# Isabella98Liu/DG-Mesh

Hardware: AMD Instinct MI355X
Metric: train-step iters/sec (800x800, ~100k Gaussians) (higher is better)
Workload: dtype f32 (f16x3p split products, fp32 accumulate); 1 GPU; D-NeRF jumpingjacks-like cfg2: 800x800, P=100000 Gaussians, deformation MLP on (deform + deform_back, is_blender), 1 frame per rank per step, fixed P (no densification inside the timed region); output heads of both networks scaled x0.01 so that the deformation field is small as after convergence (default init triples every splat's extent); P=100000, W=800, H=800, num_rendered=2808497, visible=95520, mlp_impl=hip, parallelism=dp1 (frame-parallel, flat-bucket all-reduce 27.8 MB)

## Files before the change

dg-mesh_amd/csrc/mlp.hip:

```cpp
#include <stdlib.h>
#include <string.h>

#include "dgm_common.hpp"
#include "mlp_planes.hpp"
#include "mlp_planes5.hpp"

namespace dgm {

static constexpr int MLP_W = 256;
static constexpr int MLP_EMB = 96;
static constexpr int MLP_XE = 63;
static constexpr int GM = 64, GK = 16, GAP = 66;
static constexpr int DW_ROWS = 512;
static constexpr int DW_SLAB = 128;
static constexpr int HD_ROWS = 256;

__global__ void mlp_prep_kernel(int in_features, int Kp, int emb_dim, int is_skip, const float* __restrict__ W,
                                float* __restrict__ Wt, float* __restrict__ Wd) {
    const int idx = blockIdx.x * blockDim.x + threadIdx.x;
    if (idx < Kp * MLP_W) {
        const int k = idx / MLP_W, j = idx % MLP_W;
        int src = -1;
        if (Kp == MLP_W) src = k;
        else if (k < MLP_EMB) src = k < emb_dim ? k : -1;
// ... 911 lines not shown
                dgm::prof_begin(DGM_STAGE_MLP_LAYER_FWD, st);
                P4_LAUNCH((mlp_gemm4_kernel<16, 1024, 512, 0, false, 8, true>), CfgFwdC::LDS, gx, st, a)
                dgm::prof_end(DGM_STAGE_MLP_LAYER_FWD, st);
            }
        }
    } else {
    a.A = (const unsigned char*)w.emb, a.Aexp = w.Eexp, a.Bp = w.Wt3[0], a.b_inv = w.wsc_f[0], a.bias = p->b[0];
    a.mask_out = w.mask[0], a.C = (unsigned char*)w.Y[0], a.Cexp = w.Yexp[0];
    a.Bp2 = w.Wt3[sk], a.b_inv2 = w.wsc_e, a.bias2 = p->b[sk], a.out2 = w.Cin;
    P4_LAUNCH((mlp_gemm4_kernel<6, 384, 192, 0, true, 8>), CfgL0::LDS, gx, st, a)
    a.Bp2 = nullptr, a.b_inv2 = nullptr, a.bias2 = nullptr, a.out2 = nullptr;
    for (int l = 1; l < 8; l++) {
        a.A = (const unsigned char*)w.Y[l - 1], a.Aexp = w.Yexp[l - 1], a.b_inv = w.wsc_f[l], a.bias = p->b[l];
        a.mask_out = w.mask[l], a.C = (unsigned char*)w.Y[l], a.Cexp = w.Yexp[l];
        if (l == sk) {
            a.Bp = w.Wt3[l] + (size_t)MLP_EMB * MLP_W / 4, a.cin = w.Cin;
            P4_LAUNCH((mlp_gemm4_kernel<16, 1024, 512, 2, false, 8>), CfgSkip::LDS, gx, st, a)
            a.cin = nullptr;
        } else {
            a.Bp = w.Wt3[l];
            dgm::prof_begin(DGM_STAGE_MLP_LAYER_FWD, st);
            P4_LAUNCH((mlp_gemm4_kernel<16, 1024, 512, 0, false, 8>), CfgFwd::LDS, gx, st, a)
            dgm::prof_end(DGM_STAGE_MLP_LAYER_FWD, st);
        }
    }
    }
    a.Bp2 = nullptr, a.b_inv2 = nullptr, a.bias2 = nullptr, a.out2 = nullptr, a.cin = nullptr;
    a.A = (const unsigned char*)w.Y[7], a.Aexp = w.Yexp[7], a.Bp = w.Wh4f, a.b_inv = w.wsc_hf, a.bias = p->bh;
    a.mask_out = nullptr, a.C = nullptr, a.Cexp = nullptr, a.out = out, a.ldo = p->n_out, a.n_valid = p->n_out;
    if (fold && heads_fused) {}
    else if (fold) P4_LAUNCH((mlp_gemm4_kernel<16, 1024, 512, 3, false, 1, true>), CfgHeadsC::LDS, gx, st, a)
    else P4_LAUNCH((mlp_gemm4_kernel<16, 1024, 512, 3, false, 1>), CfgHeads::LDS, gx, st, a)
    hipError_t e = hipGetLastError();
    if (e != hipSuccess) return mlp_fail(hipGetErrorString(e));
    return 0;
}

int backward_planes(const dgm_mlp_params* p, int N, const float* dOut, int temb_stride, const Ws& w, float* const* dW, float* const* db,
                    float* dWh, float* dbh, float* dtemb, hipStream_t st, const bool fold, const bool all5, const float* x_in = nullptr,
                    float* dX = nullptr) {
    const P4Plan pl = p4_plan(N);
    const int nt = pl.ntiles, gx = nt < num_cus() ? nt : num_cus();
    const int sk = p->skip_layer;
    const int EW = fold ? 64 : MLP_EMB;
    hipLaunchKernelGGL(mlp_dout4_kernel, dim3((nt + 3) / 4), dim3(256), 0, st, N, nt, p->n_out, dOut, w.Dp, w.Dexp, w.partial_hb);
    unsigned char* G = (unsigned char*)w.Ga;
    unsigned char* Gn = (unsigned char*)w.Gb;
    int *Ge = w.Gexp[0], *Gne = w.Gexp[1];
    Gemm4Args a;
    memset(&a, 0, sizeof(a));
    a.ntiles = nt, a.M = N, a.exps_limit = p4_exps_limit();
    a.A = w.Dp, a.Aexp = w.Dexp, a.Bp = w.Wh4b, a.b_inv = w.wsc_hb, a.mask_in = w.mask[7], a.C = G, a.Cexp = Ge;
    Dw4Args d;
    memset(&d, 0, sizeof(d));
    d.ntiles = nt, d.tiles_per_chunk = pl.tiles_per_chunk;
    d.X = (const unsigned char*)w.Y[7], d.Xexp = w.Yexp[7], d.G = w.Dp, d.Gexp = w.Dexp, d.partial = w.partial_h, d.chunk_stride = 0;
    d.partial_db = nullptr;
    {
        static const int mult = [] { const char* e = getenv("DGM_P4_G7_MULT"); return e ? atoi(e) : 2; }();
        const int g7 = nt < mult * num_cus() ? nt : mult * num_cus();
        if (fold) P4_LAUNCH((mlp_gemm4_kernel<1, 128, 64, 1, false, 8, true>), CfgG7C::LDS, g7, st, a)
        else P4_LAUNCH((mlp_gemm4_kernel<1, 128, 64, 1, false, 8>), CfgG7::LDS, g7, st, a)
    }
    P4_LAUNCH((mlp_dw4_kernel<8, 1, 1024, 512, 128, 64>), CfgDwH::LDS, pl.chunks, st, d)
    ReduceDwBatch rb;
    rb.emb_dim = p->emb_dim, rb.n_jobs = 0;
    int rb_blocks = 0, n_pending = 0;
    auto add_job = [&](int slot, int chunks, int db_rows, int Kp, int in_features, int dst_off, const float* partial,
                       const float* partial_db, float* dWp, float* dbp) {
        ReduceDwJob& jb = rb.job[slot];
        jb.chunks = chunks, jb.db_rows = db_rows, jb.Kp = Kp, jb.in_features = in_features, jb.nblocks = reduce_dw_blocks(Kp);
        jb.emb_rows = EW, jb.k_valid = fold ? MLP_XE : p->emb_dim;
        jb.dst_off = dst_off, jb.partial = partial, jb.partial_db = partial_db, jb.dW = dWp, jb.db = dbp;
        if (jb.nblocks > rb_blocks) rb_blocks = jb.nblocks;
    };
    int n_dw = p4_pair_split(nt, gx);
    if (n_dw > pl.chunks) n_dw = pl.chunks;
    const bool per_row_t = temb_stride != 0 && dtemb != nullptr;
    if (per_row_t && dX) return mlp_fail("mlp_backward: position gradients need a broadcast time row");
    for (int l = 7; l >= 0; l--) {
        const int Kp = l == 0 ? EW : (l == sk ? EW + MLP_W : MLP_W);
        const bool paired = n_dw > 0 && l >= 1;
        const int tpc_pair = paired ? (nt + n_dw - 1) / n_dw : 0;
        const int chunks_l = paired ? (nt + tpc_pair - 1) / tpc_pair : pl.chunks;
        if (l >= 1) {
            a.A = G, a.Aexp = Ge, a.Bp = w.Wd3[l], a.b_inv = w.wsc_d[l], a.mask_in = w.mask[l - 1], a.C = Gn, a.Cexp = Gne;
        }
        d.G = G, d.Gexp = Ge;
        if (dX && (l == sk || l == 0))
            hipLaunchKernelGGL(mlp_dx4_kernel, dim3(nt), dim3(256), 0, st, N, (const unsigned char*)G, (const int*)Ge, p->W[l],
                               layer_in(p, l), 0, MLP_XE, reinterpret_cast<float*>(w.Cin), l == 0 ? 1 : 0, x_in, dX, 0);
        if (per_row_t && (l == sk || l == 0))
            hipLaunchKernelGGL(mlp_dx4_kernel, dim3(nt), dim3(256), 0, st, N, (const unsigned char*)G, (const int*)Ge, p->W[l],
                               layer_in(p, l), MLP_XE, p->t_dim, reinterpret_cast<float*>(w.Cin), l == 0 ? 2 : 0, (const float*)nullptr,
                               dtemb, p->t_dim);
        float* part_emb = w.partial_l[l];
        float* part_trunk = w.partial_l[l] + (l == sk ? (size_t)EW * MLP_W : 0);
        size_t stride_emb = (size_t)Kp * MLP_W, stride_trunk = (size_t)Kp * MLP_W;
        if (paired && l == sk) {
            part_trunk = w.partial_l[l], stride_trunk = (size_t)MLP_W * MLP_W;
            part_emb = w.partial_l[l] + (size_t)n_dw * MLP_W * MLP_W, stride_emb = (size_t)EW * MLP_W;
        }
        if (l == 0 || l == sk) {
            d.tiles_per_chunk = pl.tiles_per_chunk;
            d.X = (const unsigned char*)w.emb, d.Xexp = w.Eexp, d.partial = part_emb, d.chunk_stride = stride_emb, d.partial_db = w.partial_db_l[l];
            if (fold) P4_LAUNCH((mlp_dw4_kernel<2, 8, 256, 128, 1024, 512>), CfgDwE64::LDS, pl.chunks, st, d)
            else P4_LAUNCH((mlp_dw4_kernel<3, 8, 384, 192, 1024, 512>), CfgDwE::LDS, pl.chunks, st, d)
        }
        if (l != 0) {
            d.tiles_per_chunk = paired ? tpc_pair : pl.tiles_per_chunk;
            d.X = (const unsigned char*)w.Y[l - 1], d.Xexp = w.Yexp[l - 1];
            d.partial = part_trunk, d.chunk_stride = stride_trunk;
            d.partial_db = l == sk ? nullptr : w.partial_db_l[l];
        }
        if (paired) {
            dgm::prof_begin(DGM_STAGE_MLP_BWD_PAIR, st);
            {
                static bool done_[DGM_MAX_DEVICES] = {false}, donec_[DGM_MAX_DEVICES] = {false};
                constexpr int LDS_PAIR = CfgBwdC::LDS > CfgDw::LDS ? CfgBwdC::LDS : CfgDw::LDS;
                if ((fold ? p4_lds_attr(mlp_bwd_pair_kernel<true>, LDS_PAIR, &donec_[current_device_slot()])
                          : p4_lds_attr(mlp_bwd_pair_kernel<false>, LDS_PAIR, &done_[current_device_slot()])) != hipSuccess)
                    return mlp_fail("mlp: cannot raise the LDS limit of mlp_bwd_pair_kernel");
                const int grid = n_dw + (gx - n_dw > 0 ? gx - n_dw : 1);
                static const int chunk_env = [] { const char* e = getenv("DGM_MLP_PAIR_CHUNKED"); return e ? atoi(e) : 1; }();
                const int chunked = (chunk_env && grid - n_dw == n_dw && (n_dw % 8) == 0) ? 1 : 0;
                if (fold) hipLaunchKernelGGL(mlp_bwd_pair_kernel<true>, dim3(grid), dim3(512), LDS_PAIR, st, a, d, n_dw, chunked);
                else hipLaunchKernelGGL(mlp_bwd_pair_kernel<false>, dim3(grid), dim3(512), LDS_PAIR, st, a, d, n_dw, chunked);
            }
            dgm::prof_end(DGM_STAGE_MLP_BWD_PAIR, st);
        } else if (l >= 1) {
            dgm::prof_begin(DGM_STAGE_MLP_LAYER_BWD, st);
            if (all5) {
                Gemm5Args b;
                memset(&b, 0, sizeof(b));
                b.ntiles = nt, b.M = N, b.exps_limit = a.exps_limit;
                b.A = a.A, b.Aexp = a.Aexp, b.Bp = a.Bp, b.b_inv = a.b_inv, b.mask_in = a.mask_in, b.C = a.C, b.Cexp = a.Cexp;
                P5_LAUNCH((mlp_gemm5_kernel<0, 1>), Cfg5Bwd::LDS, gx, st, b)
            } else if (fold)
                P4_LAUNCH((mlp_gemm4_kernel<16, 1024, 512, 1, false, 8, true>), CfgBwdC::LDS, gx, st, a)
            else
                P4_LAUNCH((mlp_gemm4_kernel<16, 1024, 512, 1, false, 8>), CfgBwd::LDS, gx, st, a)
            dgm::prof_end(DGM_STAGE_MLP_LAYER_BWD, st);
            dgm::prof_begin(DGM_STAGE_MLP_LAYER_DW, st);
            P4_LAUNCH((mlp_dw4_kernel<8, 8, 1024, 512, 1024, 512>), CfgDw::LDS, chunks_l, st, d)
            dgm::prof_end(DGM_STAGE_MLP_LAYER_DW, st);
        }
        if (paired && l == sk) {
            add_job(n_pending++, pl.chunks, 8 * pl.chunks, EW, layer_in(p, l), 0, part_emb, w.partial_db_l[l], dW[l], db[l]);
            add_job(n_pending++, chunks_l, 0, MLP_W, layer_in(p, l), p->emb_dim, part_trunk, nullptr, dW[l], nullptr);
        } else
            add_job(n_pending++, chunks_l, 8 * chunks_l, Kp, layer_in(p, l), 0, w.partial_l[l], w.partial_db_l[l], dW[l], db[l]);
        if (l >= 1) {
            unsigned char* t = G;
            G = Gn, Gn = t;
            int* te = Ge;
            Ge = Gne, Gne = te;
        }
    }
    rb.n_jobs = n_pending;
    rb.h_chunks = pl.chunks, rb.h_bchunks = nt, rb.h_nout = p->n_out, rb.h_partial_W = w.partial_h, rb.h_partial_b = w.partial_hb;
    rb.h_dW = dWh, rb.h_db = dbh;
    hipLaunchKernelGGL(mlp_reduce_dw_all_kernel, dim3(rb_blocks, rb.n_jobs + 1), dim3(256), 0, st, rb);
    if (fold) {
        FoldGradArgs f;
        f.dW[0] = dW[0], f.db[0] = db[0], f.W[0] = p->W[0], f.in_features[0] = layer_in(p, 0);
        f.dW[1] = dW[sk], f.db[1] = db[sk], f.W[1] = p->W[sk], f.in_features[1] = layer_in(p, sk);
        f.temb = w.temb_row, f.T = p->t_dim, f.dtemb = (dtemb != nullptr && !per_row_t) ? dtemb : nullptr;
        hipLaunchKernelGGL(mlp_fold_grad_kernel, dim3(f.dtemb != nullptr ? 3 : 2, p->t_dim), dim3(256), 0, st, f);
    } else if (dtemb != nullptr && !per_row_t)
        hipLaunchKernelGGL(mlp_dtemb_bcast_kernel, dim3(p->t_dim), dim3(256), 0, st, p->t_dim, db[0], p->W[0], layer_in(p, 0),
                           db[sk], p->W[sk], layer_in(p, sk), dtemb);
    hipError_t e = hipGetLastError();
    if (e != hipSuccess) return mlp_fail(hipGetErrorString(e));
    return 0;
}
}

extern "C" {

int dgm_mlp_set_gemm(int mode) {
    const int prev = g_gemm_mode;
    if (mode == 1 || mode == 3 || mode == 4 || mode == 5) g_gemm_mode = mode;
    return prev;
}

size_t dgm_mlp_workspace_bytes(int N) {
    Ws w = carve(nullptr, N > 0 ? N : 0);
    return w.bytes;
}

#ifdef P4_TIMING
int dgm_p4_timing(unsigned long long* out) {
    return (int)hipMemcpyFromSymbol(out, HIP_SYMBOL(dgm::g_p4_timing), sizeof(unsigned long long) * 256 * 8 * 16);
}
#endif

#ifdef P4_PROBE
namespace {
__global__ void p4_probe_fill_kernel(unsigned* __restrict__ p, size_t n, unsigned seed, int zero) {
    for (size_t i = blockIdx.x * (size_t)blockDim.x + threadIdx.x; i < n; i += (size_t)gridDim.x * blockDim.x) {
        unsigned x = (unsigned)i * 2654435761u + seed;
        x ^= x >> 15, x *= 0x2c1b3c6du, x ^= x >> 12;
        p[i] = zero ? 0u : (x & 0xbfffbfffu);
    }
}
}
int dgm_p4_probe(int N, int kind, int iters, int zero, void* stream) {
    hipStream_t st = (hipStream_t)stream;
    const P4Plan pl = p4_plan(N);
    const int nt = pl.ntiles, gx = nt < num_cus() ? nt : num_cus();
    static unsigned char *A = nullptr, *C = nullptr, *G = nullptr;
    static int* ex = nullptr;
    static uint4* Bp = nullptr;
    static float *binv = nullptr, *bias = nullptr, *partial = nullptr, *pdb = nullptr;
    static unsigned* mask = nullptr;
    static int cap = 0;
    const size_t rows = (size_t)nt * 32;
    if (cap < nt) {
        if (hipMalloc((void**)&A, rows * 1024) != hipSuccess || hipMalloc((void**)&C, rows * 1024) != hipSuccess ||
            hipMalloc((void**)&G, rows * 1024) != hipSuccess || hipMalloc((void**)&ex, (size_t)nt * 4 * 4) != hipSuccess ||
            hipMalloc((void**)&Bp, 16 * 4 * 256 * 16) != hipSuccess || hipMalloc((void**)&binv, 1024) != hipSuccess ||
            hipMalloc((void**)&bias, 1024) != hipSuccess || hipMalloc((void**)&mask, (size_t)nt * 1024) != hipSuccess ||
            hipMalloc((void**)&partial, (size_t)256 * 256 * 256 * 4) != hipSuccess || hipMalloc((void**)&pdb, (size_t)256 * 8 * 256 * 4) != hipSuccess)
            return mlp_fail("p4_probe: hipMalloc failed");
        cap = nt;
    }
    hipLaunchKernelGGL(p4_probe_fill_kernel, dim3(1024), dim3(256), 0, st, (unsigned*)A, rows * 256, 1u, zero);
    hipLaunchKernelGGL(p4_probe_fill_kernel, dim3(1024), dim3(256), 0, st, (unsigned*)G, rows * 256, 2u, zero);
    hipLaunchKernelGGL(p4_probe_fill_kernel, dim3(64), dim3(256), 0, st, (unsigned*)Bp, (size_t)16 * 4 * 256 * 4, 3u, zero);
    hipLaunchKernelGGL(p4_probe_fill_kernel, dim3(256), dim3(256), 0, st, mask, (size_t)nt * 256, 4u, 0);
    (void)hipMemsetAsync(ex, 0, (size_t)nt * 4 * 4, st);
    (void)hipMemsetAsync(bias, 0, 1024, st);
    const float one = 1.0f / 65536.0f;
    {
        float ones[256];
        for (int i = 0; i < 256; i++) ones[i] = one;
        (void)hipMemcpyAsync(binv, ones, sizeof(ones), hipMemcpyHostToDevice, st);
        (void)hipStreamSynchronize(st);
    }
    Gemm4Args a;
    memset(&a, 0, sizeof(a));
    a.exps_limit = 512;
    a.ntiles = nt, a.M = N, a.A = kind == 0 ? A : G, a.Aexp = ex, a.Bp = Bp, a.b_inv = binv, a.bias = bias, a.mask_in = mask,
    a.mask_out = mask + (size_t)0, a.C = C, a.Cexp = ex + nt;
    Dw4Args d;
    memset(&d, 0, sizeof(d));
    d.ntiles = nt, d.tiles_per_chunk = pl.tiles_per_chunk, d.X = A, d.Xexp = ex + 2 * nt, d.G = G, d.Gexp = ex + 3 * nt, d.partial = partial,
    d.chunk_stride = (size_t)256 * 256, d.partial_db = pdb;
    int n_dw = p4_pair_split(nt, gx);
    if (n_dw > pl.chunks) n_dw = pl.chunks;
    Gemm5Args a5;
    memset(&a5, 0, sizeof(a5));
    a5.exps_limit = 512, a5.ntiles = nt, a5.M = N, a5.A = (kind == 4) ? A : G, a5.Aexp = ex, a5.Bp = Bp, a5.b_inv = binv, a5.bias = bias;
    a5.mask_in = mask, a5.mask_out = mask, a5.C = C, a5.Cexp = ex + nt;
    for (int it = 0; it < iters; it++) {
        if (kind == 4) {
            P5_LAUNCH((mlp_gemm5_kernel<0, 0>), Cfg5Fwd::LDS, gx, st, a5)
        } else if (kind == 5) {
            P5_LAUNCH((mlp_gemm5_kernel<0, 1>), Cfg5Bwd::LDS, gx, st, a5)
        } else if (kind == 0) {
            P4_LAUNCH((mlp_gemm4_kernel<16, 1024, 512, 0, false, 8>), CfgFwd::LDS, gx, st, a)
        } else if (kind == 3) {
            P4_LAUNCH((mlp_gemm4_kernel<16, 1024, 512, 1, false, 8>), CfgBwd::LDS, gx, st, a)
        } else if (kind == 1) {
            P4_LAUNCH((mlp_dw4_kernel<8, 8, 1024, 512, 1024, 512>), CfgDw::LDS, pl.chunks, st, d)
        } else {
            if (n_dw <= 0) return mlp_fail("p4_probe: no pair split at this size");
            static bool done_[DGM_MAX_DEVICES] = {false};
            constexpr int LDS_PAIR = CfgBwd::LDS > CfgDw::LDS ? CfgBwd::LDS : CfgDw::LDS;
            if (p4_lds_attr(mlp_bwd_pair_kernel<false>, LDS_PAIR, &done_[current_device_slot()]) != hipSuccess) return mlp_fail("p4_probe: LDS attribute");
            Dw4Args dp = d;
            dp.tiles_per_chunk = (nt + n_dw - 1) / n_dw;
#ifdef P4_XCD_REDUCE
            {
                static unsigned* xs = nullptr;
                static float* xp = nullptr;
                static int gen = 0;
                if (!xs) {
                    if (hipMalloc((void**)&xs, 8 * 128) != hipSuccess || hipMalloc((void**)&xp, (size_t)8 * 65536 * 4) != hipSuccess) return mlp_fail("p4_probe: hipMalloc");
                    (void)hipMemsetAsync(xs, 0, 8 * 128, st);
                }
                dp.xsync = getenv("DGM_P4_XCD_OFF") ? nullptr : xs, dp.xpartial = xp, dp.xgen = gen++, dp.xchunks = (nt + dp.tiles_per_chunk - 1) / dp.tiles_per_chunk;
            }
#endif
            const int grid = n_dw + (gx - n_dw > 0 ? gx - n_dw : 1);
            const int chunked = (grid - n_dw == n_dw && (n_dw % 8) == 0) ? 1 : 0;
            hipLaunchKernelGGL(mlp_bwd_pair_kernel<false>, dim3(grid), dim3(512), LDS_PAIR, st, a, dp, n_dw, chunked);
        }
    }
    hipError_t e = hipGetLastError();
    if (e != hipSuccess) return mlp_fail(hipGetErrorString(e));
    return 0;
}
#endif

int dgm_mlp_describe_workspace(int N, size_t* offs, int capacity) {
    Ws w = carve(nullptr, N > 0 ? N : 0);
    const char* base = nullptr;
    const void* f[DGM_MLP_WS_FIELDS];
    int n = 0;
    f[n++] = w.emb;
    for (int l = 0; l < 8; l++) f[n++] = w.Y[l];
    for (int l = 0; l < 8; l++) f[n++] = w.mask[l];
    f[n++] = w.Ga, f[n++] = w.Gb;
    f[n++] = w.Eexp;
    for (int l = 0; l < 8; l++) f[n++] = w.Yexp[l];
    f[n++] = w.Dexp, f[n++] = w.Gexp[0], f[n++] = w.Gexp[1];
    f[n++] = w.Cin, f[n++] = w.Dp;
    for (int l = 0; l < 8; l++) f[n++] = w.partial_l[l];
    for (int l = 0; l < 8; l++) f[n++] = w.partial_db_l[l];
    for (int i = 0; i < n && i < capacity; i++) offs[i] = (size_t)((const char*)f[i] - base);
    return n;
}

int dgm_mlp_forward(const dgm_mlp_params* p, int N, const float* x, const float* temb, int temb_stride, char* workspace,
                    float* out, void* stream) {
    if (check_params(p)) return 1;
    if (N <= 0) return 0;
    if (!x || !temb || !workspace || !out) return mlp_fail("mlp_forward: NULL pointer");
    hipStream_t st = (hipStream_t)stream;
    Ws w = carve(workspace, N);
    const int mode = g_gemm_mode;
    const bool fold = (mode == 3 || mode == 5) && temb_stride == 0;
    remember_ws_mode(workspace, mode + (fold ? 16 : 0));
    if (mode >= 3) return forward_planes(p, N, x, temb, temb_stride, w, out, st, fold, fold && mode == 5);
    for (int l = 0; l < 8; l++) {
        const int Kp = layer_kp(p, l);
        const int n = (Kp > MLP_W ? Kp : MLP_W) * MLP_W;
        hipLaunchKernelGGL(mlp_prep_kernel, dim3((n + 255) / 256), dim3(256), 0, st, layer_in(p, l), Kp, p->emb_dim,
                           l == p->skip_layer ? 1 : 0, p->W[l], w.Wt[l], l >= 1 ? w.Wd[l] : nullptr);
    }
    hipLaunchKernelGGL(mlp_embed_kernel, dim3((N + 7) / 8), dim3(256), 0, st, N, x, temb, temb_stride, p->t_dim, w.emb);
    const int grid = (N + GM - 1) / GM;
    for (int l = 0; l < 8; l++) {
        const float *A1, *A2 = nullptr;
        int lda1, K1, lda2 = 0, K2 = 0;
        if (l == 0) {
            A1 = w.emb, lda1 = MLP_EMB, K1 = MLP_EMB;
        } else if (l == p->skip_layer) {
            A1 = w.emb, lda1 = MLP_EMB, K1 = MLP_EMB, A2 = w.Y[l - 1], lda2 = MLP_W, K2 = MLP_W;
        } else {
            A1 = w.Y[l - 1], lda1 = MLP_W, K1 = MLP_W;
        }
        hipLaunchKernelGGL(mlp_gemm_kernel<0>, dim3(grid, MLP_W / GN), dim3(256), 0, st, N, A1, lda1, K1, A2, lda2, K2, w.Wt[l],
                           p->b[l], w.mask[l], w.Y[l]);
    }
    hipLaunchKernelGGL(mlp_rows_small_kernel, dim3((N * 4 + 255) / 256), dim3(256), 0, st, N, p->n_out, w.Y[7], p->Wh, 1,
                       MLP_W, p->bh, out, p->n_out, 0);
    hipError_t e = hipGetLastError();
    if (e != hipSuccess) return mlp_fail(hipGetErrorString(e));
    return 0;
}

int dgm_mlp_backward(const dgm_mlp_params* p, int N, const float* dOut, int temb_stride, char* workspace, float* const* dW,
                     float* const* db, float* dWh, float* dbh, float* dtemb, void* stream) {
    return dgm_mlp_backward_dx(p, N, dOut, temb_stride, workspace, dW, db, dWh, dbh, dtemb, nullptr, nullptr, stream);
}

int dgm_mlp_backward_dx(const dgm_mlp_params* p, int N, const float* dOut, int temb_stride, char* workspace, float* const* dW,
                        float* const* db, float* dWh, float* dbh, float* dtemb, const float* x, float* dX, void* stream) {
    if (check_params(p)) return 1;
    if (N <= 0) return 0;
    if (!dOut || !workspace || !dW || !db || !dWh || !dbh) return mlp_fail("mlp_backward: NULL pointer");
    if ((x == nullptr) != (dX == nullptr)) return mlp_fail("mlp_backward: x and dX come together");
    const int mode = g_gemm_mode;
    if (dX && (mode < 3 || temb_stride != 0))
        return mlp_fail("mlp_backward: the gradient w.r.t. the positions exists in the plane arithmetic only (f16x3p, broadcast time row)");
    {
        const int fm = recall_ws_mode(workspace);
        if (fm >= 0 && (fm & 15) != mode)
// ... 84 lines not shown
```

dg-mesh_amd/csrc/mlp_planes.hpp:

```cpp
#pragma once
#include <type_traits>

#include "dgm_common.hpp"

namespace dgm {

typedef _Float16 f16x8 __attribute__((ext_vector_type(8)));
typedef _Float16 f16x2 __attribute__((ext_vector_type(2)));
typedef float f32x2 __attribute__((ext_vector_type(2)));
#ifndef DGM_F32X16_DEFINED
#define DGM_F32X16_DEFINED
typedef float f32x16 __attribute__((ext_vector_type(16)));
#endif

__device__ __forceinline__ f16x8 as_f16x8(const uint4 v) { return __builtin_bit_cast(f16x8, v); }

__device__ __forceinline__ void split2h(float a0, float a1, unsigned& h, unsigned& l) {
    const f16x2 hh = __builtin_convertvector((f32x2){a0, a1}, f16x2);
    const float r0 = a0 - (float)hh.x, r1 = a1 - (float)hh.y;
    const f16x2 ll = __builtin_convertvector((f32x2){r0, r1}, f16x2);
    h = __builtin_bit_cast(unsigned, hh);
    l = __builtin_bit_cast(unsigned, ll);
}

// ... 796 lines not shown
        if (HM.value && j + 1 < my_tiles)
            asm volatile("s_waitcnt lgkmcnt(%0)\n\ts_barrier" ::"n"((EPI == 0 ? 4 : 0) + 2 * (P4_PD < KS ? P4_PD : KS) + (COLSC ? 1 : 0)) : "memory");
        else if (HM.value && EPI == 0) asm volatile("s_waitcnt lgkmcnt(%0)\n\ts_barrier" ::"n"(4 + (COLSC ? 1 : 0)) : "memory");
        else P4_LDS_BARRIER();
        P4_T(6)
    };
    {
        const unsigned char* ps = Abuf + li * PITCH + g * 16;
#pragma unroll
        for (int i = 0; i < P4_PD && i < KS; i++) G4_FRAG(i);
    }
    typedef std::integral_constant<bool, true> T_;
    typedef std::integral_constant<bool, false> F_;
    step(T_{}, F_{}, F_{}, 0, 0);
    if (my_tiles > 1) step(T_{}, T_{}, F_{}, 1, 1);
    int ab = 2;
    for (int j = 2; j < my_tiles; j++) {
        step(T_{}, T_{}, T_{}, j, ab);
        ab = ab == 2 ? 0 : ab + 1;
    }
    if (my_tiles >= 2) step(F_{}, T_{}, T_{}, my_tiles, my_tiles % 3);
    else step(F_{}, T_{}, F_{}, my_tiles, my_tiles % 3);
    step(F_{}, F_{}, T_{}, my_tiles + 1, (my_tiles + 1) % 3);
#ifdef P4_TIMING
    if (P4_TIME_ON && lane == 0 && bx < 256) {
#pragma unroll
        for (int k = 0; k < 8; k++) g_p4_timing[(bx * 8 + wv) * 16 + k] = tacc[k];
        g_p4_timing[(bx * 8 + wv) * 16 + 8] = t_loop - t_entry;
        g_p4_timing[(bx * 8 + wv) * 16 + 9] = __builtin_amdgcn_s_memtime() - t_entry;
        g_p4_timing[(bx * 8 + wv) * 16 + 10] = t_entry;
        g_p4_timing[(bx * 8 + wv) * 16 + 11] = __builtin_amdgcn_s_memtime();
        g_p4_timing[(bx * 8 + wv) * 16 + 12] = my_tiles;
        g_p4_timing[(bx * 8 + wv) * 16 + 13] = t_p1 - t_entry;
        g_p4_timing[(bx * 8 + wv) * 16 + 14] = t_p2 - t_p1;
        g_p4_timing[(bx * 8 + wv) * 16 + 15] = t_p3 - t_p2;
    }
#endif
#undef G4_COPY
#undef G4_COPY1
#undef G4_FRAG
#undef G4_MFMA
}

template <int KS, int ROWB, int PLANEB, int EPI, bool DUAL, int NCW, bool COLSC = false>
__global__ void __launch_bounds__(512)
mlp_gemm4_kernel(const Gemm4Args a) {
    extern __shared__ __attribute__((aligned(16))) unsigned char p4_smem[];
    gemm4_body<KS, ROWB, PLANEB, EPI, DUAL, NCW, COLSC>(a, (int)blockIdx.x, (int)gridDim.x, p4_smem);
}

struct Dw4Args {
    int ntiles, tiles_per_chunk;
    const unsigned char* X;
    const int* Xexp;
    const unsigned char* G;
    const int* Gexp;
    float* partial;
    size_t chunk_stride;
    float* partial_db;
#ifdef P4_XCD_REDUCE
    unsigned* xsync;
    float* xpartial;
    int xgen, xchunks;
#endif
};

__device__ __forceinline__ int dw4_pos(int col) { return (col & ~7) | ((col ^ (col >> 3)) & 7); }
__device__ __forceinline__ unsigned dw4_dword(const uint4& v, int i) { return i == 0 ? v.x : (i == 1 ? v.y : (i == 2 ? v.z : v.w)); }
__device__ __forceinline__ float dw4_dot_ones(unsigned d, float acc) {
    const f16x2 one = {(_Float16)1.0f, (_Float16)1.0f};
    return __builtin_amdgcn_fdot2(__builtin_bit_cast(f16x2, d), one, acc, false);
}
__device__ __forceinline__ unsigned dw4_pk_mul(unsigned d, unsigned f2) {
    return __builtin_bit_cast(unsigned, __builtin_bit_cast(f16x2, d) * __builtin_bit_cast(f16x2, f2));
}

template <int MT, int NT, int XROWB, int XPLANEB, int GROWB, int GPLANEB>
struct Dw4Cfg {
    static constexpr int XK = MT * 32, GK = NT * 32;
    static constexpr int XU = 8 * XK, GU = 8 * GK;
    static constexpr int LDS = 2 * (XU + GU) * 16;
};

template <int MT, int NT, int XROWB, int XPLANEB, int GROWB, int GPLANEB>
__device__ __forceinline__ void dw4_body(const Dw4Args& a, const int chunk, unsigned char* smem) {
    using Cfg = Dw4Cfg<MT, NT, XROWB, XPLANEB, GROWB, GPLANEB>;
    constexpr int XK = Cfg::XK, GK = Cfg::GK, XU = Cfg::XU, GU = Cfg::GU;
    constexpr int XCG = XK / 8, GCG = GK / 8;
    constexpr int XB = XCG * 8, GB = GCG * 8;
    constexpr int MTW = NT == 8 ? MT : 1;
    static_assert(NT == 8 || (NT == 1 && MT == 8), "wave decomposition");
    static_assert(XB <= 256 && GB <= 256, "stager layout");
    uint4* const dw4_lds = reinterpret_cast<uint4*>(smem);
    uint4* Xs = dw4_lds;
    uint4* Gs = dw4_lds + 2 * XU;
    const int tid = threadIdx.x, lane = tid & 63, wv = __builtin_amdgcn_readfirstlane(tid >> 6);
    const int g = lane >> 5, li = lane & 31;
    const int t0 = chunk * a.tiles_per_chunk, t1 = min(a.ntiles, t0 + a.tiles_per_chunk);
    const int nst = t1 - t0;
    if (nst <= 0) return;

    int eref = 0x7fffffff;
    for (int t = t0; t < t1; t++) eref = min(eref, a.Xexp[t] + a.Gexp[t]);
    eref = __builtin_amdgcn_readfirstlane(eref);

    const bool isX = tid < XB, isG = tid >= 256 && tid < 256 + GB;
    const int st = isG ? tid - 256 : tid;
    const int ncg = isG ? GCG : XCG;
#ifndef DW4_ROWMAJOR_STAGERS
#define DW4_ROWMAJOR_STAGERS 1
#endif
    const int cg = st % ncg;
    const int pl = DW4_ROWMAJOR_STAGERS ? (st / ncg) & 1 : st / (ncg * 4);
    const int rg = DW4_ROWMAJOR_STAGERS ? st / (ncg * 2) : (st / ncg) & 3;
    const unsigned char* src = isG ? a.G + (size_t)pl * GPLANEB + cg * 16 : a.X + (size_t)pl * XPLANEB + cg * 16;
    const int srow = isG ? GROWB : XROWB;
    uint4* sdst = (isG ? Gs : Xs) + (pl * 4 + rg) * (isG ? GK : XK) + cg * 8;
    const int sbuf = isG ? GU : XU;
    const int swz = cg & 7;
    uint4 R[8];
    float cs[8];
#pragma unroll
    for (int i = 0; i < 8; i++) cs[i] = 0.f;

#define DW4_LOAD(t_)                                                                                                   \
    if (isX || isG) {                                                                                                  \
        const unsigned char* p_ = src + ((size_t)(t_) * 32 + rg * 8) * srow;                                           \
        _Pragma("unroll") for (int i_ = 0; i_ < 8; i_++) R[i_] = *reinterpret_cast<const uint4*>(p_ + (size_t)i_ * srow); \
    }
#define DW4_STORE(t_, buf_)                                                                                            \
    if (isX || isG) {                                                                                                  \
        const int et_ = a.Xexp[t_] + a.Gexp[t_];                                                                       \
        const unsigned f2_ = p4_pow2_h2(eref - et_);                                                                   \
        const bool scale_ = isX && et_ != eref;                                                                        \
        float tsum_[8];                                                                                                \
        _Pragma("unroll") for (int c_ = 0; c_ < 8; c_++) {                                                             \
            const unsigned sel_ = (c_ & 1) ? 0x07060302u : 0x05040100u;                                                \
            uint4 o_;                                                                                                  \
            o_.x = __builtin_amdgcn_perm(dw4_dword(R[1], c_ >> 1), dw4_dword(R[0], c_ >> 1), sel_);                    \
            o_.y = __builtin_amdgcn_perm(dw4_dword(R[3], c_ >> 1), dw4_dword(R[2], c_ >> 1), sel_);                    \
            o_.z = __builtin_amdgcn_perm(dw4_dword(R[5], c_ >> 1), dw4_dword(R[4], c_ >> 1), sel_);                    \
            o_.w = __builtin_amdgcn_perm(dw4_dword(R[7], c_ >> 1), dw4_dword(R[6], c_ >> 1), sel_);                    \
            if (isG && a.partial_db != nullptr) {                                                                      \
                float s_ = dw4_dot_ones(o_.x, 0.f);                                                                    \
                s_ = dw4_dot_ones(o_.y, s_), s_ = dw4_dot_ones(o_.z, s_), s_ = dw4_dot_ones(o_.w, s_);                 \
                tsum_[c_] = s_;                                                                                        \
            }                                                                                                          \
            if (scale_) o_.x = dw4_pk_mul(o_.x, f2_), o_.y = dw4_pk_mul(o_.y, f2_), o_.z = dw4_pk_mul(o_.z, f2_), o_.w = dw4_pk_mul(o_.w, f2_); \
            sdst[(buf_) * sbuf + (c_ ^ swz)] = o_;                                                                     \
        }                                                                                                              \
        if (isG && a.partial_db != nullptr) {                                                                          \
            const float ig_ = p4_pow2(-a.Gexp[t_]);                                                                    \
            _Pragma("unroll") for (int c_ = 0; c_ < 8; c_++) cs[c_] += tsum_[c_] * ig_;                                \
        }                                                                                                              \
    }

    f32x16 acc[MTW];
#pragma unroll
    for (int mt = 0; mt < MTW; mt++)
#pragma unroll
        for (int r = 0; r < 16; r++) acc[mt][r] = 0.f;

    const int gcol = NT == 8 ? wv * 32 + li : li;
    const int gpos = dw4_pos(gcol);

    DW4_LOAD(t0)
    DW4_STORE(t0, 0)
    if (nst > 1) DW4_LOAD(t0 + 1)
    __syncthreads();
    for (int s = 0; s < nst; s++) {
        const int buf = s & 1;
        if (s + 1 < nst) {
            DW4_STORE(t0 + s + 1, buf ^ 1)
            if (s + 2 < nst) DW4_LOAD(t0 + s + 2)
        }
        __builtin_amdgcn_sched_barrier(0);
        const uint4* xs = Xs + buf * XU;
        const uint4* gs = Gs + buf * GU;
#pragma unroll
        for (int kk = 0; kk < 2; kk++) {
            const int kg = 2 * kk + g;
            const f16x8 gh = as_f16x8(gs[kg * GK + gpos]), gl = as_f16x8(gs[(4 + kg) * GK + gpos]);
            if (MTW == 1) {
                const int xpos = dw4_pos(wv * 32 + li);
                const f16x8 ah = as_f16x8(xs[kg * XK + xpos]), al = as_f16x8(xs[(4 + kg) * XK + xpos]);
                acc[0] = __builtin_amdgcn_mfma_f32_32x32x16_f16(ah, gl, acc[0], 0, 0, 0);
                acc[0] = __builtin_amdgcn_mfma_f32_32x32x16_f16(al, gh, acc[0], 0, 0, 0);
                acc[0] = __builtin_amdgcn_mfma_f32_32x32x16_f16(ah, gh, acc[0], 0, 0, 0);
            } else {
#pragma unroll
                for (int mp = 0; mp < (MTW + 1) / 2; mp++) {
                    const int m0 = 2 * mp, m1 = 2 * mp + 1 < MTW ? 2 * mp + 1 : 2 * mp;
                    const int xp0 = dw4_pos(m0 * 32 + li), xp1 = dw4_pos(m1 * 32 + li);
                    const f16x8 ah0 = as_f16x8(xs[kg * XK + xp0]), al0 = as_f16x8(xs[(4 + kg) * XK + xp0]);
                    if (m1 != m0) {
                        const f16x8 ah1 = as_f16x8(xs[kg * XK + xp1]), al1 = as_f16x8(xs[(4 + kg) * XK + xp1]);
                        acc[m0] = __builtin_amdgcn_mfma_f32_32x32x16_f16(ah0, gl, acc[m0], 0, 0, 0);
                        acc[m1] = __builtin_amdgcn_mfma_f32_32x32x16_f16(ah1, gl, acc[m1], 0, 0, 0);
                        acc[m0] = __builtin_amdgcn_mfma_f32_32x32x16_f16(al0, gh, acc[m0], 0, 0, 0);
                        acc[m1] = __builtin_amdgcn_mfma_f32_32x32x16_f16(al1, gh, acc[m1], 0, 0, 0);
                        acc[m0] = __builtin_amdgcn_mfma_f32_32x32x16_f16(ah0, gh, acc[m0], 0, 0, 0);
                        acc[m1] = __builtin_amdgcn_mfma_f32_32x32x16_f16(ah1, gh, acc[m1], 0, 0, 0);
                    } else {
                        acc[m0] = __builtin_amdgcn_mfma_f32_32x32x16_f16(ah0, gl, acc[m0], 0, 0, 0);
                        acc[m0] = __builtin_amdgcn_mfma_f32_32x32x16_f16(al0, gh, acc[m0], 0, 0, 0);
                        acc[m0] = __builtin_amdgcn_mfma_f32_32x32x16_f16(ah0, gh, acc[m0], 0, 0, 0);
                    }
                }
            }
        }
        P4_LDS_BARRIER();
    }
#undef DW4_LOAD
#undef DW4_STORE

    if (NT == 8) {
        float* out = a.partial + (size_t)chunk * a.chunk_stride;
        const int col = wv * 32 + li;
#pragma unroll
        for (int mt = 0; mt < MTW; mt++) {
#pragma unroll
            for (int r = 0; r < 16; r++) {
                const int k = mt * 32 + (r & 3) + 8 * (r >> 2) + 4 * g;
                out[(size_t)k * 256 + col] = ldexpf(acc[mt][r], -eref);
            }
        }
#ifdef P4_XCD_REDUCE
        if (MT == 8 && a.xsync != nullptr) {
            const int grp = chunk & 7, member = chunk >> 3;
            const int members = (a.xchunks - grp + 7) >> 3;
            __syncthreads();
            if (tid == 0) {
                __builtin_amdgcn_fence(__ATOMIC_RELEASE, "agent");
                asm volatile("s_waitcnt vmcnt(0)" ::: "memory");
                atomicAdd(&a.xsync[grp * 32], 1u);
                const unsigned want = (unsigned)members * (unsigned)(a.xgen + 1);
                for (int spin = 0; spin < (1 << 20); spin++) {
                    if (__hip_atomic_load(&a.xsync[grp * 32], __ATOMIC_RELAXED, __HIP_MEMORY_SCOPE_AGENT) >= want) break;
                    __builtin_amdgcn_s_sleep(8);
                }
                __builtin_amdgcn_fence(__ATOMIC_ACQUIRE, "agent");
            }
            __syncthreads();
            const int rows_per = (256 + members - 1) / members, r0 = member * rows_per, r1 = min(256, r0 + rows_per);
            for (int i = r0 * 64 + tid; i < r1 * 64; i += 512) {
                float4 sacc = make_float4(0.f, 0.f, 0.f, 0.f);
                for (int m = 0; m < members; m++) {
                    const float4 v = *reinterpret_cast<const float4*>(a.partial + (size_t)(grp + 8 * m) * a.chunk_stride + (size_t)i * 4);
                    sacc.x += v.x, sacc.y += v.y, sacc.z += v.z, sacc.w += v.w;
                }
                *reinterpret_cast<float4*>(a.xpartial + ((size_t)grp * 65536 + (size_t)i * 4)) = sacc;
            }
        }
#endif
    } else {
        if (li < 16) {
#pragma unroll
            for (int r = 0; r < 16; r++) {
                const int c = wv * 32 + (r & 3) + 8 * (r >> 2) + 4 * g;
                a.partial[((size_t)chunk * 16 + li) * 256 + c] = ldexpf(acc[0][r], -eref);
            }
        }
    }
    if (isG && a.partial_db != nullptr) {
        float* d = a.partial_db + ((size_t)chunk * 8 + pl * 4 + rg) * GK + cg * 8;
        *reinterpret_cast<float4*>(d) = make_float4(cs[0], cs[1], cs[2], cs[3]);
        *reinterpret_cast<float4*>(d + 4) = make_float4(cs[4], cs[5], cs[6], cs[7]);
    }
}

template <int MT, int NT, int XROWB, int XPLANEB, int GROWB, int GPLANEB>
__global__ void __launch_bounds__(512)
mlp_dw4_kernel(const Dw4Args a) {
    extern __shared__ __attribute__((aligned(16))) unsigned char p4_smem[];
    dw4_body<MT, NT, XROWB, XPLANEB, GROWB, GPLANEB>(a, (int)blockIdx.x, p4_smem);
}

template <bool COLSC>
__global__ void __launch_bounds__(512)
mlp_bwd_pair_kernel(const Gemm4Args ga, const Dw4Args da, const int n_dw, const int chunked) {
    extern __shared__ __attribute__((aligned(16))) unsigned char p4_smem[];
    if ((int)blockIdx.x < n_dw) {
        dw4_body<8, 8, 1024, 512, 1024, 512>(da, (int)blockIdx.x, p4_smem);
    } else if (chunked) {
        const int w = (int)blockIdx.x - n_dw;
        const int first = w * da.tiles_per_chunk;
        const int cnt = min(da.tiles_per_chunk, ga.ntiles - first);
        gemm4_body<16, 1024, 512, 1, false, 8, COLSC>(ga, first, 1, p4_smem, cnt > 0 ? cnt : 0);
    } else {
        gemm4_body<16, 1024, 512, 1, false, 8, COLSC>(ga, (int)blockIdx.x - n_dw, (int)gridDim.x - n_dw, p4_smem);
    }
}

__global__ void __launch_bounds__(256)
mlp_dx4_kernel(int N, const unsigned char* __restrict__ G, const int* __restrict__ Gexp, const float* __restrict__ W, int in_features,
               int col0, int ncol, float* __restrict__ scratch, int finish, const float* __restrict__ x, float* __restrict__ dX,
               int ldo) {
    __shared__ float sG[32][32 + 1];
    __shared__ float sW[32][64 + 1];
    __shared__ float sE[32][64 + 1];
    const int tile = blockIdx.x, r0 = tile * 32, tid = threadIdx.x;
    const int ty = tid >> 4, tx = tid & 15;
    const float scale = __builtin_ldexpf(1.0f, -Gexp[tile]);
    float acc[2][4] = {{0.f, 0.f, 0.f, 0.f}, {0.f, 0.f, 0.f, 0.f}};
    for (int k0 = 0; k0 < 256; k0 += 32) {
        {
            const int r = tid >> 3, kk = (tid & 7) * 4;
            const unsigned char* row = G + (size_t)(r0 + r) * 1024;
            const uint2 h = *reinterpret_cast<const uint2*>(row + (k0 + kk) * 2);
            const uint2 l = *reinterpret_cast<const uint2*>(row + 512 + (k0 + kk) * 2);
            const f16x2 h0 = __builtin_bit_cast(f16x2, h.x), h1 = __builtin_bit_cast(f16x2, h.y);
            const f16x2 l0 = __builtin_bit_cast(f16x2, l.x), l1 = __builtin_bit_cast(f16x2, l.y);
            sG[r][kk + 0] = (float)h0[0] + (float)l0[0];
            sG[r][kk + 1] = (float)h0[1] + (float)l0[1];
            sG[r][kk + 2] = (float)h1[0] + (float)l1[0];
            sG[r][kk + 3] = (float)h1[1] + (float)l1[1];
        }
        for (int i = tid; i < 32 * 64; i += 256) {
            const int kk = i >> 6, c = i & 63;
            sW[kk][c] = c < ncol ? W[(size_t)(k0 + kk) * in_features + col0 + c] : 0.f;
        }
        __syncthreads();
#pragma unroll 8
        for (int kk = 0; kk < 32; kk++) {
            const float g0 = sG[2 * ty][kk], g1 = sG[2 * ty + 1][kk];
#pragma unroll
            for (int c = 0; c < 4; c++) {
                const float wv = sW[kk][4 * tx + c];
                acc[0][c] = fmaf(g0, wv, acc[0][c]);
                acc[1][c] = fmaf(g1, wv, acc[1][c]);
            }
        }
        __syncthreads();
    }
#pragma unroll
    for (int e = 0; e < 2; e++) {
        const int r = r0 + 2 * ty + e;
        float4 v = make_float4(acc[e][0] * scale, acc[e][1] * scale, acc[e][2] * scale, acc[e][3] * scale);
        float4* sp = reinterpret_cast<float4*>(scratch + (size_t)r * 64 + 4 * tx);
        if (finish) {
            const float4 p = *sp;
            v.x += p.x, v.y += p.y, v.z += p.z, v.w += p.w;
            sE[2 * ty + e][4 * tx + 0] = v.x, sE[2 * ty + e][4 * tx + 1] = v.y, sE[2 * ty + e][4 * tx + 2] = v.z, sE[2 * ty + e][4 * tx + 3] = v.w;
        } else {
            *sp = v;
        }
    }
    if (!finish) return;
    if (finish == 2) {
        __syncthreads();
        for (int i = tid; i < 32 * ncol; i += 256) {
            const int rl = i / ncol, c = i - rl * ncol;
            if (r0 + rl < N) dX[(size_t)(r0 + rl) * ldo + c] = sE[rl][c];
        }
        return;
    }
    __syncthreads();
    if (tid < 96) {
        const int rl = tid / 3, d = tid - 3 * rl, r = r0 + rl;
        if (r < N) {
            const float xv = x[3 * r + d];
            float g = sE[rl][d];
#pragma unroll
            for (int q = 0; q < 10; q++) {
                float sn, cs;
                const float f = (float)(1 << q);
// ... 10 lines not shown
```

Before: 318.7 it/s.

## Split paired dW blocks into column halves over doubled tile chunks

In the paired backward kernel, each dW block now computes one 128-column half of the 256x256 weight-gradient tile across two adjacent tile chunks, instead of the full 256 columns over one chunk. Two blocks share each doubled chunk, one per half, and the tiles are interleaved so that each block's loads line up with the co-scheduled dgrad blocks. This halves the number of partial dW slabs that the reduction must sum, and each block stages only half of the G columns. The cost is reading the X tiles twice, once per half, and more complex index mapping between blocks and chunks.

```diff
diff --git a/dg-mesh_amd/csrc/mlp.hip b/dg-mesh_amd/csrc/mlp.hip
--- a/dg-mesh_amd/csrc/mlp.hip
+++ b/dg-mesh_amd/csrc/mlp.hip
@@ -1017,7 +1017,8 @@
         const int Kp = l == 0 ? EW : (l == sk ? EW + MLP_W : MLP_W);
         const bool paired = n_dw > 0 && l >= 1;
         const int tpc_pair = paired ? (nt + n_dw - 1) / n_dw : 0;
-        const int chunks_l = paired ? (nt + tpc_pair - 1) / tpc_pair : pl.chunks;
+        const bool halved = paired && !all5 && (n_dw % 16) == 0;
+        const int chunks_l = paired ? (nt + (halved ? 2 : 1) * tpc_pair - 1) / ((halved ? 2 : 1) * tpc_pair) : pl.chunks;
         if (l >= 1) {
             a.A = G, a.Aexp = Ge, a.Bp = w.Wd3[l], a.b_inv = w.wsc_d[l], a.mask_in = w.mask[l - 1], a.C = Gn, a.Cexp = Gne;
         }
@@ -1059,8 +1060,9 @@
                 const int grid = n_dw + (gx - n_dw > 0 ? gx - n_dw : 1);
                 static const int chunk_env = [] { const char* e = getenv("DGM_MLP_PAIR_CHUNKED"); return e ? atoi(e) : 1; }();
                 const int chunked = (chunk_env && grid - n_dw == n_dw && (n_dw % 8) == 0) ? 1 : 0;
-                if (fold) hipLaunchKernelGGL(mlp_bwd_pair_kernel<true>, dim3(grid), dim3(512), LDS_PAIR, st, a, d, n_dw, chunked);
-                else hipLaunchKernelGGL(mlp_bwd_pair_kernel<false>, dim3(grid), dim3(512), LDS_PAIR, st, a, d, n_dw, chunked);
+                const int mode = chunked | (halved ? 2 : 0);
+                if (fold) hipLaunchKernelGGL(mlp_bwd_pair_kernel<true>, dim3(grid), dim3(512), LDS_PAIR, st, a, d, n_dw, mode);
+                else hipLaunchKernelGGL(mlp_bwd_pair_kernel<false>, dim3(grid), dim3(512), LDS_PAIR, st, a, d, n_dw, mode);
             }
             dgm::prof_end(DGM_STAGE_MLP_BWD_PAIR, st);
         } else if (l >= 1) {
@@ -1220,7 +1222,12 @@
 #endif
             const int grid = n_dw + (gx - n_dw > 0 ? gx - n_dw : 1);
             const int chunked = (grid - n_dw == n_dw && (n_dw % 8) == 0) ? 1 : 0;
-            hipLaunchKernelGGL(mlp_bwd_pair_kernel<false>, dim3(grid), dim3(512), LDS_PAIR, st, a, dp, n_dw, chunked);
+#ifdef P4_XCD_REDUCE
+            const int halved = 0;
+#else
+            const int halved = (n_dw % 16) == 0 ? 2 : 0;
+#endif
+            hipLaunchKernelGGL(mlp_bwd_pair_kernel<false>, dim3(grid), dim3(512), LDS_PAIR, st, a, dp, n_dw, chunked | halved);
         }
     }
     hipError_t e = hipGetLastError();
diff --git a/dg-mesh_amd/csrc/mlp_planes.hpp b/dg-mesh_amd/csrc/mlp_planes.hpp
--- a/dg-mesh_amd/csrc/mlp_planes.hpp
+++ b/dg-mesh_amd/csrc/mlp_planes.hpp
@@ -902,23 +902,27 @@
     static constexpr int LDS = 2 * (XU + GU) * 16;
 };
 
-template <int MT, int NT, int XROWB, int XPLANEB, int GROWB, int GPLANEB>
-__device__ __forceinline__ void dw4_body(const Dw4Args& a, const int chunk, unsigned char* smem) {
+template <int MT, int NT, int XROWB, int XPLANEB, int GROWB, int GPLANEB, bool HALF = false>
+__device__ __forceinline__ void dw4_body(const Dw4Args& a, const int chunk, unsigned char* smem, const int half = 0) {
     using Cfg = Dw4Cfg<MT, NT, XROWB, XPLANEB, GROWB, GPLANEB>;
     constexpr int XK = Cfg::XK, GK = Cfg::GK, XU = Cfg::XU, GU = Cfg::GU;
-    constexpr int XCG = XK / 8, GCG = GK / 8;
+    constexpr int GKS = HALF ? GK / 2 : GK;
+    constexpr int XCG = XK / 8, GCG = GKS / 8;
     constexpr int XB = XCG * 8, GB = GCG * 8;
-    constexpr int MTW = NT == 8 ? MT : 1;
+    constexpr int MTW = NT == 8 ? (HALF ? MT / 2 : MT) : 1;
     static_assert(NT == 8 || (NT == 1 && MT == 8), "wave decomposition");
+    static_assert(!HALF || (NT == 8 && MT == 8), "column slabs: the 256 x 256 tile only");
     static_assert(XB <= 256 && GB <= 256, "stager layout");
     uint4* const dw4_lds = reinterpret_cast<uint4*>(smem);
     uint4* Xs = dw4_lds;
     uint4* Gs = dw4_lds + 2 * XU;
     const int tid = threadIdx.x, lane = tid & 63, wv = __builtin_amdgcn_readfirstlane(tid >> 6);
     const int g = lane >> 5, li = lane & 31;
-    const int t0 = chunk * a.tiles_per_chunk, t1 = min(a.ntiles, t0 + a.tiles_per_chunk);
+    const int t0 = chunk * (HALF ? 2 : 1) * a.tiles_per_chunk, t1 = min(a.ntiles, t0 + (HALF ? 2 : 1) * a.tiles_per_chunk);
     const int nst = t1 - t0;
     if (nst <= 0) return;
+    const int n2 = HALF ? max(0, nst - a.tiles_per_chunk) : 0;
+    auto tile_at = [&](int s) { return HALF ? (s < 2 * n2 ? t0 + (s & 1) * a.tiles_per_chunk + (s >> 1) : t0 + s - n2) : t0 + s; };
 
     int eref = 0x7fffffff;
     for (int t = t0; t < t1; t++) eref = min(eref, a.Xexp[t] + a.Gexp[t]);
@@ -933,9 +937,9 @@
     const int cg = st % ncg;
     const int pl = DW4_ROWMAJOR_STAGERS ? (st / ncg) & 1 : st / (ncg * 4);
     const int rg = DW4_ROWMAJOR_STAGERS ? st / (ncg * 2) : (st / ncg) & 3;
-    const unsigned char* src = isG ? a.G + (size_t)pl * GPLANEB + cg * 16 : a.X + (size_t)pl * XPLANEB + cg * 16;
+    const unsigned char* src = isG ? a.G + (size_t)pl * GPLANEB + (HALF ? half * GKS * 2 : 0) + cg * 16 : a.X + (size_t)pl * XPLANEB + cg * 16;
     const int srow = isG ? GROWB : XROWB;
-    uint4* sdst = (isG ? Gs : Xs) + (pl * 4 + rg) * (isG ? GK : XK) + cg * 8;
+    uint4* sdst = (isG ? Gs : Xs) + (pl * 4 + rg) * (isG ? GKS : XK) + cg * 8;
     const int sbuf = isG ? GU : XU;
     const int swz = cg & 7;
     uint4 R[8];
@@ -981,18 +985,20 @@
 #pragma unroll
         for (int r = 0; r < 16; r++) acc[mt][r] = 0.f;
 
-    const int gcol = NT == 8 ? wv * 32 + li : li;
+    const int gcol = NT == 8 ? (HALF ? wv & 3 : wv) * 32 + li : li;
     const int gpos = dw4_pos(gcol);
-
-    DW4_LOAD(t0)
-    DW4_STORE(t0, 0)
-    if (nst > 1) DW4_LOAD(t0 + 1)
+    const int mb = HALF ? 4 * (wv >> 2) : 0;
+
+    DW4_LOAD(tile_at(0))
+    DW4_STORE(tile_at(0), 0)
+    if (nst > 1) DW4_LOAD(tile_at(1))
     __syncthreads();
     for (int s = 0; s < nst; s++) {
         const int buf = s & 1;
         if (s + 1 < nst) {
-            DW4_STORE(t0 + s + 1, buf ^ 1)
-            if (s + 2 < nst) DW4_LOAD(t0 + s + 2)
+            const int tn = tile_at(s + 1);
+            DW4_STORE(tn, buf ^ 1)
+            if (s + 2 < nst) DW4_LOAD(tile_at(s + 2))
         }
         __builtin_amdgcn_sched_barrier(0);
         const uint4* xs = Xs + buf * XU;
@@ -1000,7 +1006,7 @@
 #pragma unroll
         for (int kk = 0; kk < 2; kk++) {
             const int kg = 2 * kk + g;
-            const f16x8 gh = as_f16x8(gs[kg * GK + gpos]), gl = as_f16x8(gs[(4 + kg) * GK + gpos]);
+            const f16x8 gh = as_f16x8(gs[kg * GKS + gpos]), gl = as_f16x8(gs[(4 + kg) * GKS + gpos]);
             if (MTW == 1) {
                 const int xpos = dw4_pos(wv * 32 + li);
                 const f16x8 ah = as_f16x8(xs[kg * XK + xpos]), al = as_f16x8(xs[(4 + kg) * XK + xpos]);
@@ -1011,7 +1017,7 @@
 #pragma unroll
                 for (int mp = 0; mp < (MTW + 1) / 2; mp++) {
                     const int m0 = 2 * mp, m1 = 2 * mp + 1 < MTW ? 2 * mp + 1 : 2 * mp;
-                    const int xp0 = dw4_pos(m0 * 32 + li), xp1 = dw4_pos(m1 * 32 + li);
+                    const int xp0 = dw4_pos((mb + m0) * 32 + li), xp1 = dw4_pos((mb + m1) * 32 + li);
                     const f16x8 ah0 = as_f16x8(xs[kg * XK + xp0]), al0 = as_f16x8(xs[(4 + kg) * XK + xp0]);
                     if (m1 != m0) {
                         const f16x8 ah1 = as_f16x8(xs[kg * XK + xp1]), al1 = as_f16x8(xs[(4 + kg) * XK + xp1]);
@@ -1036,12 +1042,12 @@
 
     if (NT == 8) {
         float* out = a.partial + (size_t)chunk * a.chunk_stride;
-        const int col = wv * 32 + li;
+        const int col = HALF ? half * GKS + gcol : wv * 32 + li;
 #pragma unroll
         for (int mt = 0; mt < MTW; mt++) {
 #pragma unroll
             for (int r = 0; r < 16; r++) {
-                const int k = mt * 32 + (r & 3) + 8 * (r >> 2) + 4 * g;
+                const int k = (mb + mt) * 32 + (r & 3) + 8 * (r >> 2) + 4 * g;
                 out[(size_t)k * 256 + col] = ldexpf(acc[mt][r], -eref);
             }
         }
@@ -1083,7 +1089,7 @@
         }
     }
     if (isG && a.partial_db != nullptr) {
-        float* d = a.partial_db + ((size_t)chunk * 8 + pl * 4 + rg) * GK + cg * 8;
+        float* d = a.partial_db + ((size_t)chunk * 8 + pl * 4 + rg) * GK + (HALF ? half * GKS : 0) + cg * 8;
         *reinterpret_cast<float4*>(d) = make_float4(cs[0], cs[1], cs[2], cs[3]);
         *reinterpret_cast<float4*>(d + 4) = make_float4(cs[4], cs[5], cs[6], cs[7]);
     }
@@ -1098,10 +1104,19 @@
 
 template <bool COLSC>
 __global__ void __launch_bounds__(512)
-mlp_bwd_pair_kernel(const Gemm4Args ga, const Dw4Args da, const int n_dw, const int chunked) {
+mlp_bwd_pair_kernel(const Gemm4Args ga, const Dw4Args da, const int n_dw, const int mode) {
     extern __shared__ __attribute__((aligned(16))) unsigned char p4_smem[];
-    if ((int)blockIdx.x < n_dw) {
+    const int chunked = mode & 1, halved = mode & 2;
+    if ((int)blockIdx.x < n_dw && halved) {
+        const int w = (int)blockIdx.x;
+        dw4_body<8, 8, 1024, 512, 1024, 512, true>(da, 8 * (w >> 4) + (w & 7), p4_smem, (w >> 3) & 1);
+    } else if ((int)blockIdx.x < n_dw) {
         dw4_body<8, 8, 1024, 512, 1024, 512>(da, (int)blockIdx.x, p4_smem);
+    } else if (chunked && halved) {
+        const int w = (int)blockIdx.x - n_dw;
+        const int first = (2 * (8 * (w >> 4) + (w & 7)) + ((w >> 3) & 1)) * da.tiles_per_chunk;
+        const int cnt = min(da.tiles_per_chunk, ga.ntiles - first);
+        gemm4_body<16, 1024, 512, 1, false, 8, COLSC>(ga, first, 1, p4_smem, cnt > 0 ? cnt : 0);
     } else if (chunked) {
         const int w = (int)blockIdx.x - n_dw;
         const int first = w * da.tiles_per_chunk;
```

After: 288.4 it/s. 0.905x the previous value.
